# rvolden/C3POa

Hardware: AMD Instinct MI355X
Metric: R2C2 reads->consensus/sec (higher is better)
Workload: dtype int32

## Files before the change

### c3poa_amd/csrc/c3_api.hip

```cpp
#include "c3_dev.h"
#include "c3_args.h"
#include "c3_bgzf.h"
#include "c3_fastq.h"
#include "c3_inflate.h"
#include <algorithm>
#include <cstddef>
#include <cstdio>
#include <cstring>
#include <string>
#include <vector>

extern "C" void c3k_launch_conk(const ConkArgs*, int, int, int, hipStream_t);
extern "C" void c3k_launch_adapter(const AdapterArgs*, int, hipStream_t);
extern "C" void c3k_launch_pairwise(const uint8_t*, int, const uint8_t*, int, const uint8_t*, int, uint8_t*, uint8_t*, int*, hipStream_t);
extern "C" void c3k_launch_match_index(const char*, const int*, int, int, const char*, const long long*, int*, hipStream_t);
extern "C" void c3k_launch_demux(const uint8_t*, int, const uint8_t*, int, int, int, int32_t*, uint8_t*, hipStream_t);
extern "C" void c3k_launch_peaks(const PeaksArgs*, int, hipStream_t);
extern "C" int c3k_peaks_blocks_per_cu(void);
extern "C" void c3k_launch_poa(const PoaArgs*, int, int, int, hipStream_t);
extern "C" void c3k_launch_prep(const PrepArgs*, int, hipStream_t);
extern "C" void c3k_launch_window(const WinArgs*, int, hipStream_t);
extern "C" void c3k_launch_stitch(const StitchArgs*, int, hipStream_t);
extern "C" void c3k_launch_zero(const ZeroArgs*, int, hipStream_t);
extern "C" void c3k_launch_zero_long(const ZeroArgs*, int, hipStream_t);
extern "C" void c3k_launch_zero_finish(const ZeroArgs*, int, hipStream_t);
extern "C" void c3k_launch_qv(const QvArgs*, int, hipStream_t);
extern "C" int c3k_qv_lds_max(void);
extern "C" void c3k_launch_bgzf(const uint8_t*, long long, int, uint8_t*, int*, uint8_t*, hipStream_t);
extern "C" void c3k_launch_inflate(const uint8_t*, const C3BgzfMember*, int, uint8_t*, int2*, hipStream_t);
extern "C" void c3k_launch_fastq_count(const uint8_t*, uint32_t, uint32_t, int32_t*, int, C3FqHdr*, hipStream_t);
extern "C" void c3k_launch_fastq_lines(const uint8_t*, uint32_t, uint32_t, const int32_t*, int32_t*, hipStream_t);
extern "C" void c3k_launch_fastq_records(const uint8_t*, uint32_t, uint32_t, const int32_t*, int, int, int, int, int32_t*, int32_t*, long long*,
                                         C3FqHdr*, int64_t*, int64_t*, int4*, hipStream_t);
extern "C" void c3k_launch_fastq_gather(const uint8_t*, const int4*, const int64_t*, const int64_t*, long long, uint8_t*, uint8_t*, uint8_t*, hipStream_t);

__device__ __forceinline__ uint32_t pack_code(uint32_t b) {
  const uint32_t u = b & 0xDFu;
  const uint32_t c = (u >> 1) & 3u;
  const bool ok = (u == 'A') | (u == 'C') | (u == 'G') | (u == 'T') | (u == 'U');
  return ok ? (c ^ (c >> 1)) : 0u;
}
__global__ __launch_bounds__(256) void k_pack(const uint8_t* ascii, const int64_t* off, const int64_t* woff, int n, uint32_t* pk) {
  const int lane = threadIdx.x & 63;
  const int wave = (blockIdx.x * blockDim.x + threadIdx.x) >> 6, n_waves = (gridDim.x * blockDim.x) >> 6;
  for (int r = wave; r < n; r += n_waves) {
    const int64_t L = off[r + 1] - off[r];
    const int64_t nw = woff[r + 1] - woff[r];
    const uint8_t* s = ascii + off[r];
    uint32_t* dst = pk + woff[r];
    for (int64_t w = lane; w < nw; w += 64) {
      uint32_t x = 0;
      if (w * 16 + 16 <= L) {
        uint32_t v[4];
        __builtin_memcpy(v, s + w * 16, 16);
#pragma unroll
        for (int k = 0; k < 16; ++k) x |= pack_code((v[k >> 2] >> (8 * (k & 3))) & 0xFFu) << (2 * k);
      } else {
        for (int k = 0; k < 16; ++k) { int64_t i = w * 16 + k; if (i < L) x |= pack_code(s[i]) << (2 * k); }
      }
      dst[w] = x;
    }
  }
}
__global__ __launch_bounds__(256) void k_gather_cons(const char* arena, const int64_t* off, const int64_t* coff, int n, char* out) {
  const int lane = threadIdx.x & 63;
  const int wave = (blockIdx.x * blockDim.x + threadIdx.x) >> 6, n_waves = (gridDim.x * blockDim.x) >> 6;
  for (int r = wave; r < n; r += n_waves) {
    const int64_t len = coff[r + 1] - coff[r];
    const char* src = arena + off[r]; char* dst = out + coff[r];
    for (int64_t k = lane; k < len; k += 64) dst[k] = src[k];
  }
}
__device__ __forceinline__ long long cons_len_of(const C3Info* p) { return p->status == C3_ST_OK ? (long long)p->cons_len : 0; }
__global__ __launch_bounds__(256) void k_coff_sums(const C3Info* info, int n, long long* part) {
  __shared__ long long sh[256];
  const int i = blockIdx.x * 256 + threadIdx.x;
  sh[threadIdx.x] = i < n ? cons_len_of(info + i) : 0;
  __syncthreads();
  for (int d = 128; d > 0; d >>= 1) { if ((int)threadIdx.x < d) sh[threadIdx.x] += sh[threadIdx.x + d]; __syncthreads(); }
  if (threadIdx.x == 0) part[blockIdx.x] = sh[0];
}
__global__ __launch_bounds__(1024) void k_coff_scan(long long* part, int nb, int64_t* coff, int n) {
  __shared__ long long sh[1024];
  long long carry = 0;
  for (int b0 = 0; b0 < nb; b0 += 1024) {
    const int b = b0 + threadIdx.x;
    const long long v = b < nb ? part[b] : 0;
    sh[threadIdx.x] = v;
    __syncthreads();
    for (int d = 1; d < 1024; d <<= 1) { long long t = (int)threadIdx.x >= d ? sh[threadIdx.x - d] : 0; __syncthreads(); sh[threadIdx.x] += t; __syncthreads(); }
    if (b < nb) part[b] = carry + sh[threadIdx.x] - v;
    carry += sh[1023];
    __syncthreads();
  }
  if (threadIdx.x == 0) { coff[0] = 0; coff[n] = carry; }
}
// ... 29 lines not shown
static inline double dbg_now_ms() { using namespace std::chrono; return duration<double, std::milli>(steady_clock::now().time_since_epoch()).count(); }
#define DBG(...) do { if (getenv("C3_DEBUG")) { fprintf(stderr, "[c3 %.3f] ", dbg_now_ms()); fprintf(stderr, __VA_ARGS__); fflush(stderr); } } while (0)

static thread_local double g_alloc_ms = 0.0;
struct DBuf {
  void* p = nullptr; size_t cap = 0;
  DBuf() = default;
  DBuf(DBuf&& o) noexcept : p(o.p), cap(o.cap) { o.p = nullptr; o.cap = 0; }
  DBuf& operator=(DBuf&& o) noexcept { std::swap(p, o.p); std::swap(cap, o.cap); return *this; }
  DBuf(const DBuf&) = delete;
  DBuf& operator=(const DBuf&) = delete;
  ~DBuf() { if (p) (void)hipFree(p); }
  hipError_t ensure(size_t bytes) {
    if (bytes <= cap) return hipSuccess;
    const double t0 = dbg_now_ms();
    if (p) { hipError_t e = hipFree(p); p = nullptr; cap = 0; if (e != hipSuccess) return e; }
    size_t want = bytes + bytes / 8 + 256;
    hipError_t e = hipMalloc(&p, want);
    if (e == hipSuccess) cap = want;
    if (e == hipSuccess && getenv("C3_DEBUG_POISON")) e = hipMemset(p, 0xA5, want);
    g_alloc_ms += dbg_now_ms() - t0;
    return e;
  }
  template <class T> T* as() const { return (T*)p; }
};

enum { EV_N = 10 };
struct c3_handle {
  c3_config cfg; std::string err; hipStream_t stream = nullptr; int n_cus = 256; size_t mem_total = 0;
  hipStream_t stream_up = nullptr; hipEvent_t ev_up[2] = {nullptr, nullptr};
  hipStream_t stream_dn = nullptr; hipEvent_t ev_dn = nullptr; long long* h_tot = nullptr;
  std::atomic<bool> snap_pending{false}; int snap_n = 0, snap_kp = 0; long long snap_tot = 0; bool snap_cons = false;
  DBuf d_info_snap, d_coff_part;
  struct Staged { DBuf d_ascii, d_pk, d_woff, d_qual, d_off, d_strand, d_sid; std::vector<int64_t> off, woff; std::vector<int16_t> sid; std::string strand;
                  int n = 0; int64_t total = 0, words = 0, maxL = 0; bool pending = false; } st;
  hipEvent_t ev[EV_N] = {};
  int n_spl = 0, max_spl = 0; std::vector<int> sp_len; DBuf d_sp_codes, d_sp_len;
  int n = 0; int64_t total = 0, words = 0, maxL = 0; std::vector<int64_t> off, woff;
  DBuf d_ascii, d_pk, d_woff, d_qual, d_off, d_strand, d_sid, d_info, d_track, d_draft, d_tpos, d_cons, d_counter, d_gather, d_gather_off;
  DBuf d_raw, d_nraw, d_sum, d_work, d_bufA, d_bufB, d_cand, d_cst, d_msa, d_msa_off, d_msa_len;
  DBuf s_poa_i, s_poa_nk, s_poa_cells, s_poa_b, s_poa_sc, s_poa_desc, s_poa_jump, s_poa_path, d_overflow;
  int n_poa_redo = 0;
  int n_poa_redo16 = 0;
  DBuf s_eD, s_lw, d_wrec, d_wlay, d_wbase, d_wout;
  DBuf s_win_i, s_win_nk, s_win_h, s_win_d, s_win_b, s_win_sc, s_win_desc, s_win_h2, s_win_d2, d_wovf;
  DBuf s_zero_d, d_zinfo, d_zflag, d_zwork; std::vector<int> zwork;
  DBuf s_zero_l;
  DBuf d_dmx_heads, d_dmx_meta, d_dmx_out;
  DBuf d_qv, s_qv_dirs, s_qv_g, d_qv_cnt, d_gather_qv;
  hipEvent_t ev_qv[2] = {nullptr, nullptr}; c3_qv_timing qtm = {}; bool snap_qv = false;
  std::vector<Summary> sum; std::vector<int> work;
  int res_prefix = 0;
  int peaks_grid = 0; bool debug_msa = false; bool injected = false;
  int n_windows = 0;
  c3_timing tm;
  unsigned long long phase_poa[16] = {0}, phase_win[16] = {0};
  int stages_done = 0;
};

static int c3_hip_fail(c3_handle* h, hipError_t e, const char* what, int line) {
  char buf[512];
  snprintf(buf, sizeof buf, "HIP error %d (%s) at c3_api.hip:%d: %s", (int)e, hipGetErrorString(e), line, what);
  if (h) h->err = buf;
  return C3_E_HIP;
}
static int c3_fail(c3_handle* h, int code, const char* msg) { if (h) h->err = msg; return code; }

static C3Counters* dev_cnt(c3_handle* h) { return h->d_counter.as<C3Counters>(); }
template <class T> static hipError_t zero_cnt(c3_handle* h, T* field) { return hipMemsetAsync(field, 0, sizeof(T), h->stream); }
static hipError_t zero_counters(c3_handle* h) { return hipMemsetAsync(h->d_counter.p, 0, sizeof(C3Counters), h->stream); }
static hipError_t read_counters(c3_handle* h, C3Counters* c) {
  hipError_t e = hipMemcpyAsync(c, h->d_counter.p, sizeof(*c), hipMemcpyDeviceToHost, h->stream);
  return e != hipSuccess ? e : hipStreamSynchronize(h->stream);
}

extern "C" void c3_default_config(c3_config* c) {
  memset(c, 0, sizeof(*c));
  c->device = 0;
  c->conk_match = 5; c->conk_mismatch = -4; c->conk_penalty = 20;
  c->sg_iters = 3; c->sg_window = 41; c->sg_order = 2; c->mdistcutoff = 500;
  c->poa_match = 5; c->poa_mismatch = 4; c->poa_o1 = 4; c->poa_e1 = 2; c->poa_o2 = 24; c->poa_e2 = 1;
  c->poa_band_b = 10; c->poa_band_f = 0.01;
  c->pol_match = 3; c->pol_mismatch = -5; c->pol_gap = -4; c->pol_window = 500; c->pol_q = 5; c->dang_band = 128;
  c->slots_poa = 0; c->slots_win = 0; c->zero = 1; c->zero_max_cells = 16 << 20;
}
extern "C" const char* c3_version(void) { return "c3poa_amd 0.1 (gfx950)"; }
// ... 11 lines not shown
void c3_set_host_error(const char* msg) { g_create_err = msg; }

extern "C" int c3_create(const c3_config* cfg, c3_handle** out) {
  if (!cfg || !out) return C3_E_ARG;
  *out = nullptr;
  int ndev = 0;
  hipError_t e = hipGetDeviceCount(&ndev);
  if (e != hipSuccess || ndev <= 0) { g_create_err = "no HIP device: the c3poa HIP backend has no CPU fallback"; return C3_E_NO_DEVICE; }
  if (cfg->device < 0 || cfg->device >= ndev) { g_create_err = "bad device ordinal"; return C3_E_ARG; }
  if (cfg->conk_match < -127 || cfg->conk_match > 127 || cfg->conk_mismatch < -127 || cfg->conk_mismatch > 127) {
    g_create_err = "conk_match / conk_mismatch must fit a signed byte"; return C3_E_ARG;
  }
  if (cfg->sg_order != 2 && cfg->sg_order != 3) { g_create_err = "sg_order must be 2 or 3"; return C3_E_ARG; }
  if (cfg->sg_window < 5 || cfg->sg_window > 127 || !(cfg->sg_window & 1)) { g_create_err = "sg_window must be odd, 5..127"; return C3_E_ARG; }
  if (cfg->zero_max_cells < 1 || cfg->zero_max_cells > INT32_MAX) { g_create_err = "zero_max_cells must be 1..2147483647"; return C3_E_ARG; }
  c3_handle* h = new c3_handle();
  h->cfg = *cfg;
  hipDeviceProp_t prop;
  e = hipSetDevice(cfg->device);
  if (e == hipSuccess) {
    (void)hipSetDeviceFlags(hipDeviceScheduleBlockingSync); (void)hipGetLastError();
    e = hipGetDeviceProperties(&prop, cfg->device);
  }
  if (e == hipSuccess) e = hipStreamCreate(&h->stream);
  if (e == hipSuccess) e = hipStreamCreate(&h->stream_up);
  if (e == hipSuccess) e = hipStreamCreate(&h->stream_dn);
  if (e == hipSuccess) e = hipEventCreateWithFlags(&h->ev_dn, hipEventDisableTiming);
  if (e == hipSuccess) e = hipHostMalloc((void**)&h->h_tot, 64, hipHostMallocDefault);
  for (int i = 0; i < 2 && e == hipSuccess; ++i) e = hipEventCreate(&h->ev_up[i]);
  for (int i = 0; i < EV_N && e == hipSuccess; ++i) e = hipEventCreate(&h->ev[i]);
  if (e != hipSuccess) { g_create_err = hipGetErrorString(e); c3_destroy(h); return C3_E_HIP; }
  h->n_cus = prop.multiProcessorCount > 0 ? prop.multiProcessorCount : 256;
  h->mem_total = prop.totalGlobalMem;
  memset(&h->tm, 0, sizeof(h->tm));
  *out = h;
  return C3_E_OK;
}

extern "C" void c3_destroy(c3_handle* h) {
  if (!h) return;
  (void)hipSetDevice(h->cfg.device);
  for (hipStream_t s : {h->stream, h->stream_up, h->stream_dn}) if (s) (void)hipStreamSynchronize(s);
  for (hipStream_t s : {h->stream, h->stream_up, h->stream_dn}) if (s) (void)hipStreamDestroy(s);
  for (hipEvent_t ev : {h->ev_dn, h->ev_up[0], h->ev_up[1], h->ev_qv[0], h->ev_qv[1]}) if (ev) (void)hipEventDestroy(ev);
  for (hipEvent_t ev : h->ev) if (ev) (void)hipEventDestroy(ev);
  if (h->h_tot) (void)hipHostFree(h->h_tot);
  delete h;
}

static inline int code_of(char c) {
  switch (c) { case 'C': case 'c': return 1; case 'G': case 'g': return 2; case 'T': case 't': case 'U': case 'u': return 3; default: return 0; }
}

extern "C" int c3_set_splints(c3_handle* h, int n, const char* cat, const int64_t* off) {
  if (!h || n <= 0 || !cat || !off) return C3_E_ARG;
  HIPCHK(hipSetDevice(h->cfg.device));
  std::vector<uint8_t> codes((size_t)n * 2 * C3_SPLINT_MAX, 0);
  h->sp_len.assign(n, 0); h->max_spl = 0;
  for (int i = 0; i < n; ++i) {
    int S = (int)(off[i + 1] - off[i]);
    if (S <= 0 || S > C3_SPLINT_MAX) return c3_fail(h, C3_E_LIMIT, "splint length must be 1..512");
    if ((long long)std::max(h->cfg.conk_match, 0) * S > 32000 || h->cfg.conk_penalty < 0 || h->cfg.conk_penalty > 32000)
      return c3_fail(h, C3_E_LIMIT, "conk_match * splint length and conk_penalty must stay below 32000 (16-bit score cells in k_conk)");
    h->sp_len[i] = S; h->max_spl = std::max(h->max_spl, S);
    for (int k = 0; k < S; ++k) {
      int c = code_of(cat[off[i] + k]);
// ... 19 lines not shown
  C3Params p;
  p.conk_match = c.conk_match; p.conk_mismatch = c.conk_mismatch; p.conk_penalty = c.conk_penalty;
  p.sg_iters = c.sg_iters; p.sg_window = c.sg_window; p.sg_order = c.sg_order; p.mdist = c.mdistcutoff;
  p.poa_match = c.poa_match; p.poa_mismatch = c.poa_mismatch; p.o1 = c.poa_o1; p.e1 = c.poa_e1; p.o2 = c.poa_o2; p.e2 = c.poa_e2;
  p.band_b = c.poa_band_b; p.band_f = c.poa_band_f;
  p.pol_match = c.pol_match; p.pol_mismatch = c.pol_mismatch; p.pol_gap = c.pol_gap; p.pol_window = c.pol_window; p.pol_q = c.pol_q;
  p.dang_band = c.dang_band;
  p.zero = c.zero; p.zr_match = 2; p.zr_mismatch = 4; p.zr_gapo = 4; p.zr_gape = 2; p.zr_min_score = 80; p.zr_max_cells = (int)c.zero_max_cells;
  return p;
}

extern "C" int c3_batch_stage(c3_handle* h, int n, const char* seqs, const char* quals, const int64_t* off,
                              const int16_t* splint_id, const char* strand) {
  if (!h || n <= 0 || !seqs || !quals || !off || !strand) return C3_E_ARG;
  if (h->n_spl <= 0) return c3_fail(h, C3_E_STATE, "c3_set_splints must be called first");
  if (h->st.pending) return c3_fail(h, C3_E_STATE, "a staged batch is waiting for c3_batch_commit");
  HIPCHK(hipSetDevice(h->cfg.device));
  if (off[0] != 0) return c3_fail(h, C3_E_ARG, "off[0] must be 0");
  c3_handle::Staged& t = h->st;
  t.n = n; t.total = off[n] - off[0]; t.off.assign(off, off + n + 1); t.woff.assign(n + 1, 0); t.maxL = 0;
  t.sid.assign((size_t)n, 0); t.strand.assign(strand, (size_t)n);
  for (int i = 0; i < n; ++i) {
    int64_t L = off[i + 1] - off[i];
    if (L < 0 || L > (1 << 30)) return c3_fail(h, C3_E_ARG, "bad read length");
    t.maxL = std::max(t.maxL, L);
    t.woff[i + 1] = t.woff[i] + (L + 15) / 16 + 2;
    if (splint_id) { if (splint_id[i] < 0 || splint_id[i] >= h->n_spl) return c3_fail(h, C3_E_ARG, "splint_id out of range"); t.sid[i] = splint_id[i]; }
  }
  t.words = t.woff[n];
  const size_t T = (size_t)t.total;
  HIPCHK(t.d_ascii.ensure(T + 16)); HIPCHK(t.d_pk.ensure(sizeof(uint32_t) * (size_t)t.words + 64));
  HIPCHK(t.d_qual.ensure(T + 16)); HIPCHK(t.d_off.ensure(sizeof(int64_t) * (n + 1))); HIPCHK(t.d_woff.ensure(sizeof(int64_t) * (n + 1)));
  HIPCHK(t.d_strand.ensure(n)); HIPCHK(t.d_sid.ensure(sizeof(int16_t) * n));
  hipStream_t su = h->stream_up;
  HIPCHK(hipEventRecord(h->ev_up[0], su));
  HIPCHK(hipMemcpyAsync(t.d_ascii.p, seqs, T, hipMemcpyHostToDevice, su));
  HIPCHK(hipMemcpyAsync(t.d_qual.p, quals, T, hipMemcpyHostToDevice, su));
  HIPCHK(hipMemcpyAsync(t.d_off.p, t.off.data(), sizeof(int64_t) * (n + 1), hipMemcpyHostToDevice, su));
  HIPCHK(hipMemcpyAsync(t.d_woff.p, t.woff.data(), sizeof(int64_t) * (n + 1), hipMemcpyHostToDevice, su));
  HIPCHK(hipMemcpyAsync(t.d_strand.p, t.strand.data(), n, hipMemcpyHostToDevice, su));
  HIPCHK(hipMemcpyAsync(t.d_sid.p, t.sid.data(), sizeof(int16_t) * n, hipMemcpyHostToDevice, su));
  dim3 g((unsigned)std::min((n + 3) / 4, h->n_cus * 32));
  hipLaunchKernelGGL(k_pack, g, dim3(256), 0, su, t.d_ascii.as<uint8_t>(), t.d_off.as<int64_t>(), t.d_woff.as<int64_t>(), n, t.d_pk.as<uint32_t>());
  HIPCHK(hipEventRecord(h->ev_up[1], su));
  HIPCHK(hipGetLastError());
  t.pending = true;
  return C3_E_OK;
}

extern "C" int c3_batch_commit(c3_handle* h) {
  if (!h) return C3_E_ARG;
  if (!h->st.pending) return c3_fail(h, C3_E_STATE, "no staged batch");
  HIPCHK(hipSetDevice(h->cfg.device));
  HIPCHK(hipStreamSynchronize(h->stream));
  HIPCHK(hipStreamSynchronize(h->stream_up));
  c3_handle::Staged& t = h->st;
  std::swap(h->d_ascii, t.d_ascii); std::swap(h->d_pk, t.d_pk); std::swap(h->d_woff, t.d_woff); std::swap(h->d_qual, t.d_qual);
  std::swap(h->d_off, t.d_off); std::swap(h->d_strand, t.d_strand); std::swap(h->d_sid, t.d_sid);
  h->off.swap(t.off); h->woff.swap(t.woff);
  h->n = t.n; h->total = t.total; h->words = t.words; h->maxL = t.maxL;
  t.pending = false;
  const int n = h->n;
  HIPCHK(h->d_info.ensure(sizeof(C3Info) * (size_t)n));
  HIPCHK(h->d_counter.ensure(sizeof(C3Counters)));
  HIPCHK(hipMemsetAsync(h->d_info.p, 0, sizeof(C3Info) * (size_t)n, h->stream));
  hipLaunchKernelGGL(k_init_info, dim3((n + 255) / 256), dim3(256), 0, h->stream, h->d_info.as<C3Info>(), n);
  HIPCHK(hipStreamSynchronize(h->stream));
  HIPCHK(hipGetLastError());
  float ms = 0; HIPCHK(hipEventElapsedTime(&ms, h->ev_up[0], h->ev_up[1]));
  memset(&h->tm, 0, sizeof(h->tm)); h->tm.ms_pack = ms; h->tm.n_reads = n; h->tm.n_bases = h->total;
  h->stages_done = 0; h->injected = false; h->n_windows = 0; h->res_prefix = 0;
  return C3_E_OK;
}

extern "C" int c3_batch_assign(c3_handle* h, const int16_t* splint_id, const char* strand) {
  if (!h || h->n <= 0 || !splint_id || !strand) return C3_E_ARG;
  HIPCHK(hipSetDevice(h->cfg.device));
  std::vector<int16_t> sid((size_t)h->n);
  for (int i = 0; i < h->n; ++i) {
    const bool on = strand[i] == '+' || strand[i] == '-';
    if (on && (splint_id[i] < 0 || splint_id[i] >= h->n_spl)) return c3_fail(h, C3_E_ARG, "splint_id out of range");
    sid[(size_t)i] = on ? splint_id[i] : (int16_t)0;
  }
  HIPCHK(hipMemcpyAsync(h->d_strand.p, strand, (size_t)h->n, hipMemcpyHostToDevice, h->stream));
  HIPCHK(hipMemcpyAsync(h->d_sid.p, sid.data(), sizeof(int16_t) * (size_t)h->n, hipMemcpyHostToDevice, h->stream));
  hipLaunchKernelGGL(k_init_info, dim3((h->n + 255) / 256), dim3(256), 0, h->stream, h->d_info.as<C3Info>(), h->n);
  HIPCHK(hipStreamSynchronize(h->stream));
  HIPCHK(hipGetLastError());
  h->stages_done = 0;
  return C3_E_OK;
}

extern "C" int c3_batch_upload(c3_handle* h, int n, const char* seqs, const char* quals, const int64_t* off,
                               const int16_t* splint_id, const char* strand) {
  if (h && h->st.pending) { (void)hipStreamSynchronize(h->stream_up); h->st.pending = false; }
  int rc = c3_batch_stage(h, n, seqs, quals, off, splint_id, strand);
  if (rc != C3_E_OK) return rc;
  return c3_batch_commit(h);
}

static int auto_slots(c3_handle* h, int want, size_t per_slot_bytes, int n_items, int waves_per_cu) {
  int s = want > 0 ? want : h->n_cus * waves_per_cu;
  size_t budget = h->mem_total ? h->mem_total / 3 : ((size_t)64 << 30);
  if (per_slot_bytes > 0) { size_t mx = budget / per_slot_bytes; if ((size_t)s > mx) s = (int)std::max<size_t>(mx, 1); }
  if (s > n_items) s = std::max(n_items, 1);
  return s;
}

static int run_conk(c3_handle* h) {
  HIPCHK(h->d_track.ensure(sizeof(int32_t) * (size_t)h->total + 64));
  HIPCHK(zero_cnt(h, &dev_cnt(h)->queue));
  ConkArgs a; a.b = dev_batch(h); a.sp_codes = h->d_sp_codes.as<uint8_t>(); a.sp_len = h->d_sp_len.as<int>();
  a.track = h->d_track.as<int32_t>(); a.info = h->d_info.as<C3Info>(); a.cnt = dev_cnt(h);
  a.match = h->cfg.conk_match; a.mismatch = h->cfg.conk_mismatch; a.penalty = h->cfg.conk_penalty; a.n_spl = h->n_spl; a.scan = nullptr;
  int waves = std::min(h->n, h->n_cus * 32);
  c3k_launch_conk(&a, h->max_spl, (waves + 3) / 4, 0, h->stream);
  HIPCHK(hipGetLastError());
  return 0;
}

static void savgol_coeffs(int window, double* c) {
  int m = (window - 1) / 2;
  double den = (double)(2 * m - 1) * (double)(2 * m + 1) * (double)(2 * m + 3);
  for (int k = -m; k <= m; ++k) c[k + m] = 3.0 * (double)(3 * m * m + 3 * m - 1 - 5 * k * k) / den;
}

static int run_peaks(c3_handle* h) {
  static const int blocks_per_cu = c3k_peaks_blocks_per_cu();
  const int grid = std::min(h->n, h->n_cus * blocks_per_cu);
  h->peaks_grid = grid;
  const size_t mL = (size_t)h->maxL + 8;
  HIPCHK(h->d_bufA.ensure(sizeof(double) * mL * grid)); HIPCHK(h->d_bufB.ensure(sizeof(double) * mL * grid));
  HIPCHK(h->d_cand.ensure(sizeof(int32_t) * (mL / 2 + 2) * grid)); HIPCHK(h->d_cst.ensure((mL / 2 + 2) * grid));
  HIPCHK(h->d_raw.ensure(sizeof(int32_t) * (size_t)h->n * C3_MAX_PEAKS)); HIPCHK(h->d_nraw.ensure(sizeof(int32_t) * (size_t)h->n));
  PeaksArgs a; memset(&a, 0, sizeof(a));
  a.b = dev_batch(h); a.track = h->d_track.as<int32_t>(); a.info = h->d_info.as<C3Info>();
  a.bufA = h->d_bufA.as<double>(); a.bufB = h->d_bufB.as<double>(); a.cand = h->d_cand.as<int32_t>(); a.cstate = h->d_cst.as<uint8_t>();
  a.raw_peaks = h->d_raw.as<int32_t>(); a.n_raw = h->d_nraw.as<int32_t>(); a.sp_len = h->d_sp_len.as<int>();
  savgol_coeffs(h->cfg.sg_window, a.coef);
  a.maxL = (int64_t)mL; a.window = h->cfg.sg_window; a.iters = h->cfg.sg_iters; a.min_dist = h->cfg.mdistcutoff;
  a.cnt = dev_cnt(h);
  HIPCHK(zero_cnt(h, &a.cnt->peaks_queue));
  c3k_launch_peaks(&a, grid, h->stream);
  HIPCHK(hipGetLastError());
  return 0;
}

static int copy_summary(c3_handle* h) {
  const int n = h->n;
// ... 627 lines not shown
                  const char* front, const char* front_q, int front_len, const char* tail, const char* tail_q, int tail_len) {
  if (n < 1 || n > C3_MAX_SUB) return c3_fail(h, C3_E_LIMIT, "1..250 subreads");
  if (h->n_spl <= 0) { const char sp[] = "ACGT"; int64_t o[2] = {0, 4}; int rc = c3_set_splints(h, 1, sp, o); if (rc) return rc; }
  std::string seq, ql;
  c3_read_result r; memset(&r, 0, sizeof(r));
  if (front && front_len > 0) { seq.append(front, front_len); if (front_q) ql.append(front_q, front_len); else ql.append(front_len, 'I'); r.has_front = 1; r.front_end = front_len; }
  for (int i = 0; i < n; ++i) {
    r.sub_beg[i] = (int)seq.size(); seq.append(subs[i], lens[i]);
    if (quals && quals[i]) ql.append(quals[i], lens[i]); else ql.append(lens[i], 'I');
    r.sub_end[i] = (int)seq.size();
  }
  r.n_sub = n; r.n_peaks = n + 1; r.status = C3_ST_OK;
  if (tail && tail_len > 0) { r.has_tail = 1; r.tail_beg = (int)seq.size(); seq.append(tail, tail_len); if (tail_q) ql.append(tail_q, tail_len); else ql.append(tail_len, 'I'); }
  int64_t off[2] = {0, (int64_t)seq.size()};
  int16_t sid = 0; char st = '+';
  int rc = c3_batch_upload(h, 1, seq.data(), ql.data(), off, &sid, &st);
  if (rc) return rc;
  HIPCHK(hipMemcpy(h->d_info.p, &r, sizeof(r), hipMemcpyHostToDevice));
  h->injected = true;
  return 0;
}

extern "C" int c3_scan_splints(c3_handle* h, int32_t* out , int16_t* assign_splint, char* assign_strand) {
  if (!h || h->n <= 0 || h->n_spl <= 0) return C3_E_STATE;
  HIPCHK(hipSetDevice(h->cfg.device));
  const size_t items = (size_t)h->n * h->n_spl * 2;
  DBuf scan;
  HIPCHK(scan.ensure(sizeof(int32_t) * 4 * items));
  HIPCHK(zero_cnt(h, &dev_cnt(h)->queue));
  ConkArgs a; memset(&a, 0, sizeof(a));
  a.b = dev_batch(h); a.sp_codes = h->d_sp_codes.as<uint8_t>(); a.sp_len = h->d_sp_len.as<int>();
  a.track = nullptr; a.info = h->d_info.as<C3Info>(); a.cnt = dev_cnt(h);
  a.match = h->cfg.conk_match; a.mismatch = h->cfg.conk_mismatch; a.penalty = h->cfg.conk_penalty;
  a.n_spl = h->n_spl; a.scan = scan.as<int32_t>();
  const int waves = (int)std::min<size_t>(items, (size_t)h->n_cus * 32);
  c3k_launch_conk(&a, h->max_spl, (waves + 3) / 4, 1, h->stream);
  HIPCHK(hipGetLastError());
  std::vector<int32_t> tmp(4 * items);
  HIPCHK(hipMemcpyAsync(tmp.data(), scan.p, sizeof(int32_t) * 4 * items, hipMemcpyDeviceToHost, h->stream));
  HIPCHK(hipStreamSynchronize(h->stream));
  if (out) memcpy(out, tmp.data(), sizeof(int32_t) * 4 * items);
  for (int i = 0; i < h->n; ++i) {
    int best = -1, bs = -1;
    for (int c = 0; c < h->n_spl * 2; ++c) { const int32_t* e = &tmp[((size_t)i * h->n_spl * 2 + c) * 4]; if (e[0] > bs) { bs = e[0]; best = c; } }
    const long long floor51 = (long long)h->cfg.conk_match * 51 * 52 / 2;
    bool ok = best >= 0 && bs >= floor51 && (long long)bs >= 6LL * tmp[((size_t)i * h->n_spl * 2 + best) * 4 + 2];
    if (assign_splint) assign_splint[i] = ok ? (int16_t)(best >> 1) : (int16_t)-1;
    if (assign_strand) assign_strand[i] = ok ? ((best & 1) ? '-' : '+') : '?';
  }
  return C3_E_OK;
}

extern "C" int c3_scan_adapters(c3_handle* h, int32_t* out) {
  if (!h || h->n <= 0 || h->n_spl <= 0 || !out) return C3_E_STATE;
  HIPCHK(hipSetDevice(h->cfg.device));
  const size_t items = (size_t)h->n * h->n_spl * 2;
  const long long dcap = (long long)(h->maxL + 1) * (h->max_spl + 1) + 64;
  const int grid = (int)std::min<size_t>(items, (size_t)h->n_cus * 16);
  DBuf res, dd;
  HIPCHK(res.ensure(sizeof(int32_t) * 12 * items)); HIPCHK(dd.ensure((size_t)dcap * grid));
  HIPCHK(zero_cnt(h, &dev_cnt(h)->queue));
  AdapterArgs a; memset(&a, 0, sizeof(a));
  a.b = dev_batch(h); a.p = dev_params(h->cfg); a.cnt = dev_cnt(h);
  a.ad_codes = h->d_sp_codes.as<uint8_t>(); a.ad_len = h->d_sp_len.as<int>(); a.n_ad = h->n_spl;
  a.D = dd.as<uint8_t>(); a.dcap = dcap; a.out = res.as<int32_t>();
  c3k_launch_adapter(&a, grid, h->stream);
  HIPCHK(hipGetLastError());
  HIPCHK(hipMemcpyAsync(out, res.p, sizeof(int32_t) * 12 * items, hipMemcpyDeviceToHost, h->stream));
  HIPCHK(hipStreamSynchronize(h->stream));
// ... 588 lines not shown
```

### c3poa_amd/csrc/c3_args.h

```cpp
#pragma once
#include "c3_dev.h"
#include <cstddef>

struct C3Counters {
  int queue;
  int peaks_queue;
  unsigned long long cells;
  unsigned long long cells_computed;
  unsigned long long zero_cells;
  int poa_ovf;
  int poa_ovf16;
  int n_windows;
  int win_ovf;
  int win_queue2;
  int band_layers, band_fallback;
  int band_mismatch;
  struct { int window, layer, R, q, band_row, full_row, next_row; } verify;
  unsigned long long phases[16];
};
static_assert(offsetof(C3Counters, cells) % 8 == 0 && offsetof(C3Counters, cells_computed) % 8 == 0 &&
              offsetof(C3Counters, zero_cells) % 8 == 0 && offsetof(C3Counters, phases) % 8 == 0, "u64 counters must be 8-byte aligned");

struct ConkArgs {
  C3Batch b; const uint8_t* sp_codes; const int* sp_len; int32_t* track; C3Info* info; C3Counters* cnt;
  int match, mismatch, penalty;
  int n_spl; int32_t* scan;
};
struct PeaksArgs {
  C3Batch b; const int32_t* track; C3Info* info; double* bufA; double* bufB; int32_t* cand; uint8_t* cstate;
  int32_t* raw_peaks; int32_t* n_raw; const int* sp_len; double coef[64]; int64_t maxL; int window, iters, min_dist;
  C3Counters* cnt;
};
struct PoaArgs {
  C3Batch b; C3Info* info; C3Params p; C3Counters* cnt; const int* work; int n_work;
  int* ibase; int* ebase; char* cellsb; uint8_t* bbase; long long* score;
  int Ncap, K, Pcap, cells_cap;
  uint8_t* draft; int32_t* tpos; uint8_t* msa_dbg; const int64_t* msa_off; int* msa_len;
  int rb_span;
  int no2col;
  uint4* desc; int* jump;
  int* pbase;
  int* overflow;
  int* overflow16;
};
#define C3_POA_NI 19
__host__ __device__ inline int c3_poa_far_shift(bool w32) { return w32 ? 0 : 2; }
struct PoaLayout { size_t ints, edges, cells, bases, score, desc, jump, path, total; };
__host__ __device__ inline PoaLayout c3_poa_layout(size_t Ncap, size_t K, int cells_cap, int far_shift, size_t Pcap) {
  PoaLayout l;
  l.ints = sizeof(int) * C3_POA_NI * Ncap; l.edges = sizeof(int) * 3 * Ncap * K;
  l.cells = 2 * (size_t)cells_cap + 16 * (size_t)(cells_cap >> far_shift);
  l.bases = 5 * Ncap; l.score = sizeof(long long) * Ncap; l.desc = sizeof(uint4) * 2 * Ncap;
  l.jump = sizeof(int) * C3_JUMP_LEVELS * Ncap; l.path = sizeof(int) * Pcap;
  l.total = l.ints + l.edges + l.cells + l.bases + l.score + l.desc + l.jump + l.path;
  return l;
}

struct WLayer { int qbeg, len, begin, end; };
struct WinRec { int rid, w, n_layers, blen, tgs, out_len, polished, pad_; };
// ... 61 lines not shown
```

### c3poa_amd/csrc/k_conk.hip

```cpp
#include "c3_dev.h"
#include "c3_args.h"


template <int R, bool CHECK>
__device__ __forceinline__ void conk_step(int rc8, bool kill, int (&hprev)[R], int (&P)[R], int& W,
                                          int& up_prev, const int (&tbl)[R], int penalty) {
  int up = wave_shr1z(hprev[R - 1]);
  int recv = wave_shr1z(W);
  int u = up, d = up_prev;
  up_prev = up;
#pragma unroll
  for (int k = 0; k < R; ++k) {
    int s = __builtin_amdgcn_sbfe(tbl[k], rc8, 8);
    int m = max16(u, hprev[k]) - penalty;
    int hh = max16(max16(d + s, m), 0);
    if (CHECK) hh = kill ? 0 : hh;
    d = hprev[k];
    hprev[k] = hh;
    u = hh;
  }
  int wn = P[R - 1];
#pragma unroll
  for (int k = R - 1; k >= 1; --k) P[k] = P[k - 1] + hprev[k];
  P[0] = recv + hprev[0];
  W = wn;
}

template <int R, bool SCAN>
__global__ __launch_bounds__(256) void k_conk(ConkArgs a) {
  const int lane = wave_lane();
  const int n_items = SCAN ? a.b.n * a.n_spl * 2 : a.b.n;
  for (;;) {
    int item = 0;
    if (lane == 0) item = atomicAdd(&a.cnt->queue, 1);
    item = wave_first(item);
    if (item >= n_items) break;
    const int rid = SCAN ? item / (a.n_spl * 2) : item;
    const int64_t off = a.b.off[rid];
    const int L = (int)(a.b.off[rid + 1] - off);
    const int st = SCAN ? ((item & 1) ? '-' : '+') : a.b.strand[rid];
    if (!SCAN && st != '+' && st != '-') { a.info[rid].status = C3_ST_NOT_ASSIGNED; continue; }
    if (!SCAN) a.info[rid].status = C3_ST_OK;
    const int sid = SCAN ? (item >> 1) % a.n_spl : a.b.splint_id[rid];
    const int S = a.sp_len[sid];
    const uint8_t* sp = a.sp_codes + ((size_t)sid * 2 + (st == '-')) * C3_SPLINT_MAX;
    const uint32_t* pk = a.b.pk + a.b.woff[rid];
    const int last_word = L > 0 ? (L - 1) >> 4 : 0;
    int32_t* track = a.track + off;
    const int pad = 64 * R - S;
    const int mm4 = (a.mismatch & 255) * 0x01010101;
    int tbl[R], hprev[R], P[R];
#pragma unroll
    for (int k = 0; k < R; ++k) {
      int i = lane * R + k - pad;
      int code = (i >= 0) ? (int)sp[i] : 5;
      tbl[k] = code < 4 ? (mm4 & ~(255 << (8 * code))) | ((a.match & 255) << (8 * code)) : mm4;
      hprev[k] = 0; P[k] = 0;
    }
    int W = 0, up_prev = 0;
    int pen = a.penalty;
    asm volatile("" : "+v"(pen));
    int smax = -1, sarg = 0; long long ssum = 0;
    const int c0 = 63 * (R + 1) + (R - 1) - pad;
    const int T_end = L + c0;
    for (int t0 = 0; t0 < T_end; t0 += 16) {
      const bool fast = (t0 >= 63) && (t0 + 15 < L);
      const int jb = t0 - lane;
      const int wi = jb >> 4;
      const uint32_t w0 = pk[min(max(wi, 0), last_word)], w1 = pk[min(max(wi + 1, 0), last_word)];
      const uint32_t x = __builtin_amdgcn_alignbit(w1, w0, (jb & 15) * 2);
      const int d0 = t0 - c0;
      int o[16];
      if (fast) {
#pragma unroll
        for (int s = 0; s < 16; ++s) {
          const int rc8 = s >= 2 ? (int)((x >> (2 * s - 3)) & 24) : (int)((x << (3 - 2 * s)) & 24);
          conk_step<R, false>(rc8, false, hprev, P, W, up_prev, tbl, pen);
          o[s] = P[R - 1];
          if (SCAN) { int d = d0 + s; if (d >= 0 && d < L) { ssum += P[R - 1]; if (P[R - 1] > smax) { smax = P[R - 1]; sarg = d; } } }
        }
      } else {
#pragma unroll
        for (int s = 0; s < 16; ++s) {
          const int rc8 = s >= 2 ? (int)((x >> (2 * s - 3)) & 24) : (int)((x << (3 - 2 * s)) & 24);
          const bool oob = (unsigned)(jb + s) >= (unsigned)L;
          conk_step<R, true>(rc8, oob, hprev, P, W, up_prev, tbl, pen);
          o[s] = P[R - 1];
          if (SCAN) { int d = d0 + s; if (d >= 0 && d < L) { ssum += P[R - 1]; if (P[R - 1] > smax) { smax = P[R - 1]; sarg = d; } } }
        }
      }
      if (!SCAN && lane == 63) {
        if (d0 >= 0 && d0 + 15 < L) {
#pragma unroll
          for (int s = 0; s < 16; ++s) track[d0 + s] = o[s];
        } else {
#pragma unroll
          for (int s = 0; s < 16; ++s) if (d0 + s >= 0 && d0 + s < L) track[d0 + s] = o[s];
        }
      }
    }
    if (SCAN) {
      const int mean = (int)(ssum / (L > 0 ? L : 1));
      int4 v = make_int4(__builtin_amdgcn_readlane(smax, 63), __builtin_amdgcn_readlane(sarg, 63),
                         __builtin_amdgcn_readlane(mean, 63), L);
      *reinterpret_cast<int4*>(a.scan + (size_t)item * 4) = v;
    }
  }
}

extern "C" void c3k_launch_conk(const ConkArgs* a, int max_splint, int grid, int scan, hipStream_t stream) {
  int R = (max_splint + 63) / 64;
  dim3 g(grid), b(256);
#define LC(r) if (scan) hipLaunchKernelGGL((k_conk<r, true>), g, b, 0, stream, *a); else hipLaunchKernelGGL((k_conk<r, false>), g, b, 0, stream, *a); break;
  switch (R) {
    case 1: LC(1) case 2: LC(2) case 3: LC(3) case 4: LC(4) case 5: LC(5) case 6: LC(6) case 7: LC(7)
    default: LC(8)
  }
#undef LC
}
```

Measured before the change: 415,600.

## Sort reads by length and allow sub-wave lane groups in conk kernel

Adds a GPU counting sort of reads in descending length bucket order, computed on the upload stream, and makes the conk kernel process reads in that order. It also templates the kernel on a lane-group size G so one wavefront can align several reads at once, and sizes the grid from an occupancy query instead of a fixed 32 waves per CU. The default G stays 64, so the main change in effect is length-sorted scheduling plus the new grid sizing. This adds three small kernels and a memset per batch upload, and one extra indirection per work item.

```diff
diff --git a/c3poa_amd/csrc/c3_api.hip b/c3poa_amd/csrc/c3_api.hip
--- a/c3poa_amd/csrc/c3_api.hip
+++ b/c3poa_amd/csrc/c3_api.hip
@@ -10,7 +10,7 @@
 #include <string>
 #include <vector>
 
-extern "C" void c3k_launch_conk(const ConkArgs*, int, int, int, hipStream_t);
+extern "C" void c3k_launch_conk(const ConkArgs*, int, long long, int, int, int, hipStream_t);
 extern "C" void c3k_launch_adapter(const AdapterArgs*, int, hipStream_t);
 extern "C" void c3k_launch_pairwise(const uint8_t*, int, const uint8_t*, int, const uint8_t*, int, uint8_t*, uint8_t*, int*, hipStream_t);
 extern "C" void c3k_launch_match_index(const char*, const int*, int, int, const char*, const long long*, int*, hipStream_t);
@@ -62,6 +62,29 @@
     }
   }
 }
+#define C3_ORDER_BUCKETS 2048
+__device__ __forceinline__ int order_bucket(const int64_t* off, int i) {
+  const int64_t k = (off[i + 1] - off[i]) >> 6;
+  return C3_ORDER_BUCKETS - 1 - (int)(k < C3_ORDER_BUCKETS - 1 ? k : C3_ORDER_BUCKETS - 1);
+}
+__global__ __launch_bounds__(256) void k_order_hist(const int64_t* off, int n, int* hist) {
+  const int i = blockIdx.x * 256 + threadIdx.x;
+  if (i < n) atomicAdd(&hist[order_bucket(off, i)], 1);
+}
+__global__ __launch_bounds__(1024) void k_order_scan(int* hist) {
+  static_assert(C3_ORDER_BUCKETS == 2048, "one block of 1024 threads scans two buckets per thread");
+  __shared__ int sh[1024];
+  const int t = threadIdx.x, c0 = hist[2 * t], c1 = hist[2 * t + 1];
+  sh[t] = c0 + c1;
+  __syncthreads();
+  for (int d = 1; d < 1024; d <<= 1) { const int v = t >= d ? sh[t - d] : 0; __syncthreads(); sh[t] += v; __syncthreads(); }
+  const int first = sh[t] - (c0 + c1);
+  hist[2 * t] = first; hist[2 * t + 1] = first + c0;
+}
+__global__ __launch_bounds__(256) void k_order_scatter(const int64_t* off, int n, int* next, int* order) {
+  const int i = blockIdx.x * 256 + threadIdx.x;
+  if (i < n) order[atomicAdd(&next[order_bucket(off, i)], 1)] = i;
+}
 __global__ __launch_bounds__(256) void k_gather_cons(const char* arena, const int64_t* off, const int64_t* coff, int n, char* out) {
   const int lane = threadIdx.x & 63;
   const int wave = (blockIdx.x * blockDim.x + threadIdx.x) >> 6, n_waves = (gridDim.x * blockDim.x) >> 6;
@@ -157,12 +180,12 @@
   hipStream_t stream_dn = nullptr; hipEvent_t ev_dn = nullptr; long long* h_tot = nullptr;
   std::atomic<bool> snap_pending{false}; int snap_n = 0, snap_kp = 0; long long snap_tot = 0; bool snap_cons = false;
   DBuf d_info_snap, d_coff_part;
-  struct Staged { DBuf d_ascii, d_pk, d_woff, d_qual, d_off, d_strand, d_sid; std::vector<int64_t> off, woff; std::vector<int16_t> sid; std::string strand;
+  struct Staged { DBuf d_ascii, d_pk, d_woff, d_qual, d_off, d_strand, d_sid, d_order, d_obkt; std::vector<int64_t> off, woff; std::vector<int16_t> sid; std::string strand;
                   int n = 0; int64_t total = 0, words = 0, maxL = 0; bool pending = false; } st;
   hipEvent_t ev[EV_N] = {};
   int n_spl = 0, max_spl = 0; std::vector<int> sp_len; DBuf d_sp_codes, d_sp_len;
   int n = 0; int64_t total = 0, words = 0, maxL = 0; std::vector<int64_t> off, woff;
-  DBuf d_ascii, d_pk, d_woff, d_qual, d_off, d_strand, d_sid, d_info, d_track, d_draft, d_tpos, d_cons, d_counter, d_gather, d_gather_off;
+  DBuf d_ascii, d_pk, d_woff, d_qual, d_off, d_strand, d_sid, d_order, d_info, d_track, d_draft, d_tpos, d_cons, d_counter, d_gather, d_gather_off;
   DBuf d_raw, d_nraw, d_sum, d_work, d_bufA, d_bufB, d_cand, d_cst, d_msa, d_msa_off, d_msa_len;
   DBuf s_poa_i, s_poa_nk, s_poa_cells, s_poa_b, s_poa_sc, s_poa_desc, s_poa_jump, s_poa_path, d_overflow;
   int n_poa_redo = 0;
@@ -177,6 +200,7 @@
   std::vector<Summary> sum; std::vector<int> work;
   int res_prefix = 0;
   int peaks_grid = 0; bool debug_msa = false; bool injected = false;
+  int conk_g = 0;
   int n_windows = 0;
   c3_timing tm;
   unsigned long long phase_poa[16] = {0}, phase_win[16] = {0};
@@ -254,6 +278,7 @@
   if (e != hipSuccess) { g_create_err = hipGetErrorString(e); c3_destroy(h); return C3_E_HIP; }
   h->n_cus = prop.multiProcessorCount > 0 ? prop.multiProcessorCount : 256;
   h->mem_total = prop.totalGlobalMem;
+  if (const char* e_ = getenv("C3_DEBUG_CONK_G")) { const int g = atoi(e_); if (g == 16 || g == 32 || g == 64) h->conk_g = g; }
   memset(&h->tm, 0, sizeof(h->tm));
   *out = h;
   return C3_E_OK;
@@ -339,6 +364,7 @@
   HIPCHK(t.d_ascii.ensure(T + 16)); HIPCHK(t.d_pk.ensure(sizeof(uint32_t) * (size_t)t.words + 64));
   HIPCHK(t.d_qual.ensure(T + 16)); HIPCHK(t.d_off.ensure(sizeof(int64_t) * (n + 1))); HIPCHK(t.d_woff.ensure(sizeof(int64_t) * (n + 1)));
   HIPCHK(t.d_strand.ensure(n)); HIPCHK(t.d_sid.ensure(sizeof(int16_t) * n));
+  HIPCHK(t.d_order.ensure(sizeof(int) * (size_t)n)); HIPCHK(t.d_obkt.ensure(sizeof(int) * C3_ORDER_BUCKETS));
   hipStream_t su = h->stream_up;
   HIPCHK(hipEventRecord(h->ev_up[0], su));
   HIPCHK(hipMemcpyAsync(t.d_ascii.p, seqs, T, hipMemcpyHostToDevice, su));
@@ -349,6 +375,10 @@
   HIPCHK(hipMemcpyAsync(t.d_sid.p, t.sid.data(), sizeof(int16_t) * n, hipMemcpyHostToDevice, su));
   dim3 g((unsigned)std::min((n + 3) / 4, h->n_cus * 32));
   hipLaunchKernelGGL(k_pack, g, dim3(256), 0, su, t.d_ascii.as<uint8_t>(), t.d_off.as<int64_t>(), t.d_woff.as<int64_t>(), n, t.d_pk.as<uint32_t>());
+  HIPCHK(hipMemsetAsync(t.d_obkt.p, 0, sizeof(int) * C3_ORDER_BUCKETS, su));
+  hipLaunchKernelGGL(k_order_hist, dim3((n + 255) / 256), dim3(256), 0, su, t.d_off.as<int64_t>(), n, t.d_obkt.as<int>());
+  hipLaunchKernelGGL(k_order_scan, dim3(1), dim3(1024), 0, su, t.d_obkt.as<int>());
+  hipLaunchKernelGGL(k_order_scatter, dim3((n + 255) / 256), dim3(256), 0, su, t.d_off.as<int64_t>(), n, t.d_obkt.as<int>(), t.d_order.as<int>());
   HIPCHK(hipEventRecord(h->ev_up[1], su));
   HIPCHK(hipGetLastError());
   t.pending = true;
@@ -363,7 +393,7 @@
   HIPCHK(hipStreamSynchronize(h->stream_up));
   c3_handle::Staged& t = h->st;
   std::swap(h->d_ascii, t.d_ascii); std::swap(h->d_pk, t.d_pk); std::swap(h->d_woff, t.d_woff); std::swap(h->d_qual, t.d_qual);
-  std::swap(h->d_off, t.d_off); std::swap(h->d_strand, t.d_strand); std::swap(h->d_sid, t.d_sid);
+  std::swap(h->d_off, t.d_off); std::swap(h->d_strand, t.d_strand); std::swap(h->d_sid, t.d_sid); std::swap(h->d_order, t.d_order);
   h->off.swap(t.off); h->woff.swap(t.woff);
   h->n = t.n; h->total = t.total; h->words = t.words; h->maxL = t.maxL;
   t.pending = false;
@@ -420,8 +450,8 @@
   ConkArgs a; a.b = dev_batch(h); a.sp_codes = h->d_sp_codes.as<uint8_t>(); a.sp_len = h->d_sp_len.as<int>();
   a.track = h->d_track.as<int32_t>(); a.info = h->d_info.as<C3Info>(); a.cnt = dev_cnt(h);
   a.match = h->cfg.conk_match; a.mismatch = h->cfg.conk_mismatch; a.penalty = h->cfg.conk_penalty; a.n_spl = h->n_spl; a.scan = nullptr;
-  int waves = std::min(h->n, h->n_cus * 32);
-  c3k_launch_conk(&a, h->max_spl, (waves + 3) / 4, 0, h->stream);
+  a.order = h->d_order.as<int>();
+  c3k_launch_conk(&a, h->max_spl, h->n, h->n_cus, 0, h->conk_g, h->stream);
   HIPCHK(hipGetLastError());
   return 0;
 }
@@ -1115,9 +1145,8 @@
   a.b = dev_batch(h); a.sp_codes = h->d_sp_codes.as<uint8_t>(); a.sp_len = h->d_sp_len.as<int>();
   a.track = nullptr; a.info = h->d_info.as<C3Info>(); a.cnt = dev_cnt(h);
   a.match = h->cfg.conk_match; a.mismatch = h->cfg.conk_mismatch; a.penalty = h->cfg.conk_penalty;
-  a.n_spl = h->n_spl; a.scan = scan.as<int32_t>();
-  const int waves = (int)std::min<size_t>(items, (size_t)h->n_cus * 32);
-  c3k_launch_conk(&a, h->max_spl, (waves + 3) / 4, 1, h->stream);
+  a.n_spl = h->n_spl; a.scan = scan.as<int32_t>(); a.order = h->d_order.as<int>();
+  c3k_launch_conk(&a, h->max_spl, (long long)items, h->n_cus, 1, h->conk_g, h->stream);
   HIPCHK(hipGetLastError());
   std::vector<int32_t> tmp(4 * items);
   HIPCHK(hipMemcpyAsync(tmp.data(), scan.p, sizeof(int32_t) * 4 * items, hipMemcpyDeviceToHost, h->stream));
diff --git a/c3poa_amd/csrc/c3_args.h b/c3poa_amd/csrc/c3_args.h
--- a/c3poa_amd/csrc/c3_args.h
+++ b/c3poa_amd/csrc/c3_args.h
@@ -25,6 +25,7 @@
   C3Batch b; const uint8_t* sp_codes; const int* sp_len; int32_t* track; C3Info* info; C3Counters* cnt;
   int match, mismatch, penalty;
   int n_spl; int32_t* scan;
+  const int* order;
 };
 struct PeaksArgs {
   C3Batch b; const int32_t* track; C3Info* info; double* bufA; double* bufB; int32_t* cand; uint8_t* cstate;
diff --git a/c3poa_amd/csrc/k_conk.hip b/c3poa_amd/csrc/k_conk.hip
--- a/c3poa_amd/csrc/k_conk.hip
+++ b/c3poa_amd/csrc/k_conk.hip
@@ -1,12 +1,21 @@
 #include "c3_dev.h"
 #include "c3_args.h"
+#include <algorithm>
 
+#define C3_CONK_DEFAULT_G(fits16) 64
 
-template <int R, bool CHECK>
+template <int G>
+__device__ __forceinline__ int group_shr1z(int v, int gmask) {
+  if (G == 16) return __builtin_amdgcn_update_dpp(0, v, 0x111, 0xf, 0xf, true);
+  if (G == 32) return wave_shr1z(v) & gmask;
+  return wave_shr1z(v);
+}
+
+template <int G, int R, bool CHECK>
 __device__ __forceinline__ void conk_step(int rc8, bool kill, int (&hprev)[R], int (&P)[R], int& W,
-                                          int& up_prev, const int (&tbl)[R], int penalty) {
-  int up = wave_shr1z(hprev[R - 1]);
-  int recv = wave_shr1z(W);
+                                          int& up_prev, const int (&tbl)[R], int penalty, int gmask) {
+  int up = group_shr1z<G>(hprev[R - 1], gmask);
+  int recv = group_shr1z<G>(W, gmask);
   int u = up, d = up_prev;
   up_prev = up;
 #pragma unroll
@@ -26,33 +35,47 @@
   W = wn;
 }
 
-template <int R, bool SCAN>
+template <int G>
+__device__ __forceinline__ int group_last(int v, int grp) {
+  int r = __builtin_amdgcn_readlane(v, G - 1);
+#pragma unroll
+  for (int g = 1; g < 64 / G; ++g) { const int x = __builtin_amdgcn_readlane(v, g * G + G - 1); r = grp == g ? x : r; }
+  return r;
+}
+
+template <int G, int R, bool SCAN>
 __global__ __launch_bounds__(256) void k_conk(ConkArgs a) {
-  const int lane = wave_lane();
-  const int n_items = SCAN ? a.b.n * a.n_spl * 2 : a.b.n;
+  constexpr int NG = 64 / G;
+  const int lane = wave_lane(), gl = lane & (G - 1), grp = lane / G;
+  const int gmask = gl ? -1 : 0;
+  const int per_read = SCAN ? a.n_spl * 2 : 1;
+  const int n_items = a.b.n * per_read;
   for (;;) {
-    int item = 0;
-    if (lane == 0) item = atomicAdd(&a.cnt->queue, 1);
-    item = wave_first(item);
-    if (item >= n_items) break;
-    const int rid = SCAN ? item / (a.n_spl * 2) : item;
+    int base = 0;
+    if (lane == 0) base = atomicAdd(&a.cnt->queue, NG);
+    base = wave_first(base);
+    if (base >= n_items) break;
+    const int e = min(base + grp, n_items - 1);
+    const int rid = a.order[SCAN ? e / per_read : e];
+    const int sub = SCAN ? e % per_read : 0;
+    const size_t item = SCAN ? (size_t)rid * per_read + sub : (size_t)rid;
     const int64_t off = a.b.off[rid];
-    const int L = (int)(a.b.off[rid + 1] - off);
-    const int st = SCAN ? ((item & 1) ? '-' : '+') : a.b.strand[rid];
-    if (!SCAN && st != '+' && st != '-') { a.info[rid].status = C3_ST_NOT_ASSIGNED; continue; }
-    if (!SCAN) a.info[rid].status = C3_ST_OK;
-    const int sid = SCAN ? (item >> 1) % a.n_spl : a.b.splint_id[rid];
+    const int st = SCAN ? ((sub & 1) ? '-' : '+') : a.b.strand[rid];
+    const bool on = SCAN || st == '+' || st == '-';
+    if (!SCAN) a.info[rid].status = on ? C3_ST_OK : C3_ST_NOT_ASSIGNED;
+    const int L = on ? (int)(a.b.off[rid + 1] - off) : 0;
+    const int sid = SCAN ? sub >> 1 : a.b.splint_id[rid];
     const int S = a.sp_len[sid];
     const uint8_t* sp = a.sp_codes + ((size_t)sid * 2 + (st == '-')) * C3_SPLINT_MAX;
     const uint32_t* pk = a.b.pk + a.b.woff[rid];
     const int last_word = L > 0 ? (L - 1) >> 4 : 0;
     int32_t* track = a.track + off;
-    const int pad = 64 * R - S;
+    const int pad = G * R - S;
     const int mm4 = (a.mismatch & 255) * 0x01010101;
     int tbl[R], hprev[R], P[R];
 #pragma unroll
     for (int k = 0; k < R; ++k) {
-      int i = lane * R + k - pad;
+      int i = gl * R + k - pad;
       int code = (i >= 0) ? (int)sp[i] : 5;
       tbl[k] = code < 4 ? (mm4 & ~(255 << (8 * code))) | ((a.match & 255) << (8 * code)) : mm4;
       hprev[k] = 0; P[k] = 0;
@@ -61,11 +84,14 @@
     int pen = a.penalty;
     asm volatile("" : "+v"(pen));
     int smax = -1, sarg = 0; long long ssum = 0;
-    const int c0 = 63 * (R + 1) + (R - 1) - pad;
-    const int T_end = L + c0;
-    for (int t0 = 0; t0 < T_end; t0 += 16) {
-      const bool fast = (t0 >= 63) && (t0 + 15 < L);
-      const int jb = t0 - lane;
+    const int c0 = (G - 1) * (R + 1) + (R - 1) - pad;
+    const int T_end = L > 0 ? L + c0 : 0;
+    int T_max = __builtin_amdgcn_readlane(T_end, 0);
+#pragma unroll
+    for (int g = 1; g < NG; ++g) T_max = max(T_max, __builtin_amdgcn_readlane(T_end, g * G));
+    for (int t0 = 0; t0 < T_max; t0 += 16) {
+      const bool fast = (t0 >= G - 1) && __all((t0 + 15 < L) | (t0 >= T_end));
+      const int jb = t0 - gl;
       const int wi = jb >> 4;
       const uint32_t w0 = pk[min(max(wi, 0), last_word)], w1 = pk[min(max(wi + 1, 0), last_word)];
       const uint32_t x = __builtin_amdgcn_alignbit(w1, w0, (jb & 15) * 2);
@@ -75,7 +101,7 @@
 #pragma unroll
         for (int s = 0; s < 16; ++s) {
           const int rc8 = s >= 2 ? (int)((x >> (2 * s - 3)) & 24) : (int)((x << (3 - 2 * s)) & 24);
-          conk_step<R, false>(rc8, false, hprev, P, W, up_prev, tbl, pen);
+          conk_step<G, R, false>(rc8, false, hprev, P, W, up_prev, tbl, pen, gmask);
           o[s] = P[R - 1];
           if (SCAN) { int d = d0 + s; if (d >= 0 && d < L) { ssum += P[R - 1]; if (P[R - 1] > smax) { smax = P[R - 1]; sarg = d; } } }
         }
@@ -84,12 +110,12 @@
         for (int s = 0; s < 16; ++s) {
           const int rc8 = s >= 2 ? (int)((x >> (2 * s - 3)) & 24) : (int)((x << (3 - 2 * s)) & 24);
           const bool oob = (unsigned)(jb + s) >= (unsigned)L;
-          conk_step<R, true>(rc8, oob, hprev, P, W, up_prev, tbl, pen);
+          conk_step<G, R, true>(rc8, oob, hprev, P, W, up_prev, tbl, pen, gmask);
           o[s] = P[R - 1];
           if (SCAN) { int d = d0 + s; if (d >= 0 && d < L) { ssum += P[R - 1]; if (P[R - 1] > smax) { smax = P[R - 1]; sarg = d; } } }
         }
       }
-      if (!SCAN && lane == 63) {
+      if (!SCAN && gl == G - 1) {
         if (d0 >= 0 && d0 + 15 < L) {
 #pragma unroll
           for (int s = 0; s < 16; ++s) track[d0 + s] = o[s];
@@ -101,20 +127,56 @@
     }
     if (SCAN) {
       const int mean = (int)(ssum / (L > 0 ? L : 1));
-      int4 v = make_int4(__builtin_amdgcn_readlane(smax, 63), __builtin_amdgcn_readlane(sarg, 63),
-                         __builtin_amdgcn_readlane(mean, 63), L);
-      *reinterpret_cast<int4*>(a.scan + (size_t)item * 4) = v;
+      int4 v = make_int4(group_last<G>(smax, grp), group_last<G>(sarg, grp), group_last<G>(mean, grp), L);
+      *reinterpret_cast<int4*>(a.scan + item * 4) = v;
     }
   }
 }
 
-extern "C" void c3k_launch_conk(const ConkArgs* a, int max_splint, int grid, int scan, hipStream_t stream) {
-  int R = (max_splint + 63) / 64;
-  dim3 g(grid), b(256);
-#define LC(r) if (scan) hipLaunchKernelGGL((k_conk<r, true>), g, b, 0, stream, *a); else hipLaunchKernelGGL((k_conk<r, false>), g, b, 0, stream, *a); break;
-  switch (R) {
-    case 1: LC(1) case 2: LC(2) case 3: LC(3) case 4: LC(4) case 5: LC(5) case 6: LC(6) case 7: LC(7)
-    default: LC(8)
+template <int G, int R, bool SCAN>
+static void conk_launch(const ConkArgs* a, long long n_items, int n_cus, hipStream_t stream) {
+  static const int per_cu = [] {
+    int nb = 0;
+    if (hipOccupancyMaxActiveBlocksPerMultiprocessor(&nb, k_conk<G, R, SCAN>, 256, 0) != hipSuccess || nb < 1) { (void)hipGetLastError(); nb = 4; }
+    return nb;
+  }();
+  const long long waves = (n_items + 64 / G - 1) / (64 / G);
+  const long long grid = std::max<long long>(1, std::min<long long>((waves + 3) / 4, (long long)n_cus * per_cu));
+  hipLaunchKernelGGL((k_conk<G, R, SCAN>), dim3((unsigned)grid), dim3(256), 0, stream, *a);
+}
+template <int G, int R>
+static void conk_launch(const ConkArgs* a, long long n_items, int n_cus, int scan, hipStream_t stream) {
+  if (scan) conk_launch<G, R, true>(a, n_items, n_cus, stream); else conk_launch<G, R, false>(a, n_items, n_cus, stream);
+}
+
+#define C3_CONK_RMAX16 20
+#define C3_CONK_RMAX32 16
+#define C3_CONK_RMAX64 8
+static_assert(64 * C3_CONK_RMAX64 >= C3_SPLINT_MAX && 32 * C3_CONK_RMAX32 >= C3_SPLINT_MAX, "a mapping must hold the longest splint");
+
+extern "C" int c3k_conk_group(int max_splint, int force_g) {
+  const bool fits16 = (max_splint + 15) / 16 <= C3_CONK_RMAX16;
+  if (force_g == 64) return 64;
+  if (force_g == 32) return 32;
+  if (force_g == 16) return fits16 ? 16 : 32;
+  return C3_CONK_DEFAULT_G(fits16);
+}
+
+extern "C" void c3k_launch_conk(const ConkArgs* a, int max_splint, long long n_items, int n_cus, int scan, int force_g, hipStream_t stream) {
+  const int G = c3k_conk_group(max_splint, force_g);
+  const int R = (max_splint + G - 1) / G;
+#define LC(g, r) case r: conk_launch<g, r>(a, n_items, n_cus, scan, stream); break;
+  if (G == 16) switch (R) {
+    LC(16, 1) LC(16, 2) LC(16, 3) LC(16, 4) LC(16, 5) LC(16, 6) LC(16, 7) LC(16, 8) LC(16, 9) LC(16, 10)
+    LC(16, 11) LC(16, 12) LC(16, 13) LC(16, 14) LC(16, 15) LC(16, 16) LC(16, 17) LC(16, 18) LC(16, 19)
+    default: conk_launch<16, 20>(a, n_items, n_cus, scan, stream);
+  } else if (G == 32) switch (R) {
+    LC(32, 1) LC(32, 2) LC(32, 3) LC(32, 4) LC(32, 5) LC(32, 6) LC(32, 7) LC(32, 8) LC(32, 9) LC(32, 10)
+    LC(32, 11) LC(32, 12) LC(32, 13) LC(32, 14) LC(32, 15)
+    default: conk_launch<32, 16>(a, n_items, n_cus, scan, stream);
+  } else switch (R) {
+    LC(64, 1) LC(64, 2) LC(64, 3) LC(64, 4) LC(64, 5) LC(64, 6) LC(64, 7)
+    default: conk_launch<64, 8>(a, n_items, n_cus, scan, stream);
   }
 #undef LC
 }
```

Result: no change. 413,200 (-0.6%).
